# JerryX1110/Robust-Video-Object-Segmentation

Hardware: AMD Instinct MI355X
Metric: frames/sec, AOC-Net matching + calibration hot path (480p, 3 objects) (higher is better)
Workload: dtype f32; 1 GPU; cfg2: 121x213 stride-4 maps (480p), O=4 (3 objects + background), K=16 proxies, C=100, 60-frame clips, MEM_EVERY=5 (pool R=1..12), 20 Lloyd iterations, local windows 2..12, 10 IA gates + 4 conditioning blocks; sequences_per_gpu=2, proxy_mode=reference

## Files before the change

include/aoc_hip.h:

```cpp
#ifndef AOC_HIP_H
#define AOC_HIP_H

#include <stddef.h>
#include <stdint.h>

#ifdef __cplusplus
extern "C" {
#endif

typedef void *aoc_stream_t;

enum aoc_status {
    AOC_OK = 0,
    AOC_ERR_INVALID_ARG = -1,
    AOC_ERR_WORKSPACE = -2,
    AOC_ERR_LAUNCH = -3,
    AOC_ERR_UNSUPPORTED = -4
};

#define AOC_MAX_OBJECTS 30
#define AOC_MAX_CHANNELS 256
#define AOC_MAX_CLUSTERS 64
#define AOC_PAD_DISTANCE 5.0e4f
#define AOC_ROW_KEPT_BIT 0x80000000u
// ... 149 lines not shown
                              int transform, void *workspace, size_t workspace_bytes, aoc_stream_t stream);
int aoc_dense_match_min_split_cached(const float *query, const void *query_rec, const float *query_sqnorm, int query_rec_tiled,
                              int64_t m, int C, const float *pool, const void *pool_rec,
                              const int32_t *overflow_flag, int64_t n,
                              const uint32_t *right_bits, const uint32_t *wrong_bits,
                              const int32_t *fg_rows, const int32_t *obj_rows,
                              const int32_t *counts, const int32_t *obj_offsets,
                              const float *obj_bias, int n_obj,
                              float *out, int64_t out_pixel_stride, int64_t out_obj_stride,
                              int transform, void *workspace, size_t workspace_bytes, int reuse_plan, aoc_stream_t stream);

int aoc_dense_prune_stats(uint64_t *out4, int reset);
int aoc_dense_prune_stats_ex(uint64_t *out8, int reset);

int aoc_set_stream_cus(int n_cus);

int aoc_dense_match_set_probe(void *start_event, void *stop_event);

int aoc_local_window_match(const float *query, const float *prev, const uint32_t *right_bits,
                           int H, int W, int C, const int32_t *radii_host, int n_radii,
                           const float *obj_bias, int n_obj, float *out, int transform,
                           aoc_stream_t stream);

int aoc_local_window_match_ex(const float *query, const float *prev, const uint32_t *right_bits,
                              int H, int W, int C, const int32_t *radii_host, int n_radii,
                              const float *obj_bias, int n_obj, float *out, int transform,
                              int atrous_rate, int float16, aoc_stream_t stream);

int aoc_resize_bilinear_hwc(const float *in, int h, int w, int C, float *out, int H, int W,
                            aoc_stream_t stream);
// ... 332 lines not shown
```

robust-video-object-segmentation_amd/_lib.py:

```python
import ctypes
import os
import subprocess

_HERE = os.path.dirname(os.path.abspath(__file__))
CSRC = os.path.join(_HERE, "csrc")
RELEASE_SO = os.path.join(CSRC, "libaoc_hip.so")
if os.environ.get("AOC_LIB_VARIANT", "release") != "release":
    raise ImportError(f"AOC_LIB_VARIANT={os.environ['AOC_LIB_VARIANT']!r}: the development build and its switches are gone (commit fb2052a is the last "
                      "one that has them); unset the variable, or load a variant library of your own with AOC_LIB_FILE")
SO_PATH = RELEASE_SO
if os.environ.get("AOC_LIB_FILE"):
    SO_PATH = os.path.join(CSRC, os.environ["AOC_LIB_FILE"])

_vp, _i, _i64, _sz, _f = ctypes.c_void_p, ctypes.c_int, ctypes.c_int64, ctypes.c_size_t, ctypes.c_float

SIGNATURES = {
    "aoc_version": (ctypes.c_char_p, []),
    "aoc_label_prep_workspace_bytes": (_sz, [_i64, _i]),
    "aoc_label_prep": (_i, [_vp, _i64, _i, _vp, _vp, _vp, _vp, _vp, _vp, _vp, _sz, _vp]),
    "aoc_label_bits": (_i, [_vp, _i64, _i, _vp, _vp, _vp]),
    "aoc_kmeans_plan": (_i, [_vp, _i, _i, _vp, _vp]),
    "aoc_kmeans_init_rows_draw": (_i, [_vp, _vp, _vp, _i, _vp, _i, _i, _i, _vp, _vp]),
    "aoc_kmeans_workspace_bytes": (_sz, [_i64, _i, _i, _i]),
    "aoc_kmeans_segmented": (_i, [_vp, _i, _vp, _vp, _vp, _vp, _i, _i, _i, _i64, _vp, _vp, _vp, _vp, _sz, _vp]),
# ... 14 lines not shown
    "aoc_kmeans_replicate_levels": (_i, [_vp, _vp, _i, _i, _vp, _i, _i64, _vp, _vp, _vp, _vp]),
    "aoc_build_proxies_workspace_bytes": (_sz, [_i64, _i, _i]),
    "aoc_build_proxies": (_i, [_vp, _i64, _i, _vp, _vp, _vp, _vp, _vp, _i, _i, _i64, _vp, _vp, _vp, _sz, _vp]),
    "aoc_proxy_corr_min": (_i, [_vp, _i64, _i, _vp, _vp, _i, _i, _vp, _vp, _vp, _vp, _vp, _i64, _i, _vp]),
    "aoc_proxy_corr_min_batched_workspace_bytes": (_sz, []),
    "aoc_proxy_corr_min_batched": (_i, [_vp, _i, _i64, _i, _i, _i, _vp, _vp, _vp, _i, _i, _vp, _sz, _vp]),
    "aoc_proxy_corr_min_records": (_i, [_vp, _i, _i64, _i, _i, _i, _vp, _vp, _vp, _i, _vp, _sz, _vp]),
    "aoc_proxy_corr_min_records_cached_workspace_bytes": (_sz, []),
    "aoc_proxy_corr_min_records_cached": (_i, [_vp, _i, _i64, _i, _i, _i, _vp, _vp, _vp, _i, _vp, _sz, _vp, _vp]),
    "aoc_dense_match_workspace_bytes": (_sz, [_i64, _i64, _i]),
    "aoc_dense_match_min": (_i, [_vp, _i64, _i, _vp, _vp, _vp, _i64, _vp, _vp, _i, _vp, _i64, _i64, _i, _vp, _sz, _vp]),
    "aoc_dense_match_min_f16": (_i, [_vp, _i64, _i, _vp, _vp, _vp, _i64, _vp, _vp, _i, _vp, _i64, _i64, _i, _vp, _sz, _vp]),
    "aoc_proxy_corr_min_f16": (_i, [_vp, _i64, _i, _vp, _vp, _i, _i, _vp, _vp, _vp, _vp, _vp, _i64, _i, _vp]),
    "aoc_dense_match_set_probe": (_i, [_vp, _vp]),
    "aoc_set_stream_cus": (_i, [_i]),
    "aoc_split_record_bytes": (_sz, [_i]),
    "aoc_split_rows": (_i, [_vp, _i64, _i, _vp, _vp, _vp, _vp]),
    "aoc_split_rows_tiled_bytes": (_sz, [_i64, _i]),
    "aoc_split_rows_tiled": (_i, [_vp, _i64, _i, _vp, _vp, _vp, _vp]),
    "aoc_dense_match_split_workspace_bytes": (_sz, [_i64, _i64, _i]),
    "aoc_dense_prune_stats": (_i, [_vp, _i]),
    "aoc_dense_prune_stats_ex": (_i, [_vp, _i]),
    "aoc_dense_match_min_split": (_i, [_vp, _vp, _vp, _i, _i64, _i, _vp, _vp, _vp, _i64, _vp, _vp, _vp, _vp, _vp, _vp, _vp, _i, _vp, _i64, _i64, _i,
                                       _vp, _sz, _vp]),
    "aoc_dense_match_min_split_cached": (_i, [_vp, _vp, _vp, _i, _i64, _i, _vp, _vp, _vp, _i64, _vp, _vp, _vp, _vp, _vp, _vp, _vp, _i, _vp, _i64, _i64, _i,
                                              _vp, _sz, _i, _vp]),
    "aoc_frame_channels": (_i, [_i, _i, _i]),
    "aoc_frame_workspace_bytes": (_sz, [_i, _i, _i, _i, _i, _i, _i]),
    "aoc_frame_enqueue": (_i, [_vp, _vp, _vp, _sz, _vp]),
    "aoc_cluster_chain_workspace_bytes": (_sz, [_vp]),
# ... 136 lines not shown
```

robust-video-object-segmentation_amd/csrc/dense_split.hip:

```cpp
#include <atomic>
#include <type_traits>

#include "aoc_common.h"

namespace {

typedef _Float16 f16x8 __attribute__((ext_vector_type(8)));
typedef float f32x16 __attribute__((ext_vector_type(16)));

constexpr int SP_KS = 7;
constexpr int SP_K = SP_KS * 16;
constexpr int SP_HALF = SP_KS * 2;
constexpr int SP_REC = 2 * SP_HALF;
constexpr int SP_NORM_SLOT = 100;
constexpr float SP_SCALE = 1024.0f;
constexpr float SP_QCONST = 32768.0f;
constexpr float SP_UNSCALE = -1.0f / 524288.0f;
constexpr int SP_TILE = 32;
constexpr int SP_NB_HI = 8;
constexpr int SP_NQ = 2;
constexpr int SP_NW = 8;
constexpr int64_t SP_ROWS_PER_BLOCK = SP_NW * SP_NQ * 32;

static_assert(SP_NORM_SLOT + 4 <= SP_K && SP_NORM_SLOT / 16 == SP_KS - 1 && (SP_NORM_SLOT % 16) + 4 <= 8, "norm slots live in the low half of the last k-step");
// ... 180 lines not shown
constexpr int SP_CHUNK_BYTES = SP_NB_HI * SP_TILE_BYTES;
constexpr int SP_IDS_SLOTS = 3, SP_IDS_SLOT_BYTES = 1024;
constexpr int SP_IDS_OFF = SP_NBUF * SP_CHUNK_BYTES;
constexpr int SP_OBJ_OFF = SP_IDS_OFF + SP_IDS_SLOTS * SP_IDS_SLOT_BYTES;
constexpr int SP_BND_OFF = SP_OBJ_OFF + 4 * 256;
constexpr int SP_LDS_BYTES = SP_BND_OFF + SP_NW * SP_NQ * 256;
static_assert(SP_NQ == 2 && SP_NW == 8 && SP_NB_HI == 8 && SP_LDS_BYTES == 122880,
              "the step structure of dense_prune_kernel is written for 8 hi-plane tiles x 2 query tiles x 8 waves; 120 KiB per workgroup");
constexpr int SP_TILE_SLACK = 2;

template <int PLACE>
__global__ __launch_bounds__(SP_NW * 64, 1) void dense_prune_kernel(const uint4 *__restrict__ qrec, const float *__restrict__ q2, int64_t m,
                                                                     const uint4 *__restrict__ prec, const int32_t *__restrict__ tile_rows,
                                                                     const int32_t *__restrict__ tile_obj, const int32_t *__restrict__ n_tiles_ptr,
                                                                     const int32_t *__restrict__ gate, const uint32_t *__restrict__ pmax_bits,
                                                                     int n_obj, uint32_t *__restrict__ gbest, int q_tiled) {
    if (*gate) return;
    extern __shared__ __attribute__((aligned(16))) uint4 lds4[];
    constexpr int SWZ_MASK = 1;
    constexpr int SP_DMA_PER_WAVE = SP_CHUNK_BYTES / 1024 / SP_NW;
    constexpr int W_ID0 = SP_NW / 2, W_OBJ = 1;
    const uint32_t lds_base = (uint32_t)reinterpret_cast<uintptr_t>(lds4);
    const char *lds_bytes = reinterpret_cast<const char *>(lds4);

    int bx, by;
    {
        const int nb = gridDim.x * gridDim.y, lin = blockIdx.y * gridDim.x + blockIdx.x;
        const int xcd = lin & 7, slot = lin >> 3, q = nb >> 3, r = nb & 7;
        const int v = (xcd < r ? xcd * (q + 1) : r * (q + 1) + (xcd - r) * q) + slot;
        by = v / gridDim.x;
        bx = v - by * gridDim.x;
    }
    const int n_tiles = *n_tiles_ptr;
    const int ns = gridDim.y;
    if (by >= n_tiles) return;
    const int n_mine = (n_tiles - by + ns - 1) / ns;
    const int n_chunks = (n_mine + SP_NB_HI - 1) / SP_NB_HI;

    const int lane = aoc_lane(), wave = __builtin_amdgcn_readfirstlane(threadIdx.x >> 6);
    const int col = lane & 31, h = lane >> 5;
    const int64_t wave_row0 = (int64_t)bx * (SP_NW * SP_NQ * 32) + (int64_t)wave * (SP_NQ * 32);

    const float pmax = sqrtf(__uint_as_float(*pmax_bits)) * 1.001f;
    const float plmax = __uint_as_float(*(pmax_bits - 2));
    f16x8 bh[SP_NQ][SP_KS], bl[SP_NQ][SP_KS];
    float eps[SP_NQ];
    bool valid[SP_NQ];
#pragma unroll
    for (int iq = 0; iq < SP_NQ; ++iq) {
        const int64_t row = wave_row0 + iq * 32 + col;
        valid[iq] = row < m;
        const int64_t rr = valid[iq] ? row : 0;
        const uint4 *r = q_tiled ? qrec + (size_t)(rr >> 5) * (2 * SP_KS * 64) + h * 32 + (rr & 31) : qrec + (size_t)rr * SP_REC + h;
        const int ks_step = q_tiled ? 64 : 2, plane_step = q_tiled ? SP_KS * 64 : SP_HALF;
#pragma unroll
        for (int ks = 0; ks < SP_KS; ++ks) {
            uint4 u = r[ks * ks_step], v = r[plane_step + ks * ks_step];
            if (!valid[iq]) { u = make_uint4(0, 0, 0, 0); v = make_uint4(0, 0, 0, 0); }
            bh[iq][ks] = __builtin_bit_cast(f16x8, u);
            bl[iq][ks] = __builtin_bit_cast(f16x8, v);
        }
        const float ql_own = (float)bh[iq][SP_KS - 1][SP_NORM_SLOT % 16 + 3];
        if (h == 0) {
            bh[iq][SP_KS - 1][SP_NORM_SLOT % 16 + 3] = (_Float16)0.0f;
            bh[iq][SP_KS - 1][SP_NORM_SLOT % 16] = (_Float16)SP_QCONST;
            bh[iq][SP_KS - 1][SP_NORM_SLOT % 16 + 1] = (_Float16)SP_QCONST;
            bh[iq][SP_KS - 1][SP_NORM_SLOT % 16 + 2] = (_Float16)SP_QCONST;
        } else {
            bh[iq][SP_KS - 1][0] = (_Float16)0.0f;
            bh[iq][SP_KS - 1][1] = (_Float16)0.0f;
        }
        const float qn = valid[iq] ? sqrtf(q2[row]) : 0.0f;
        const float ql = valid[iq] ? __shfl(ql_own, col) : 0.0f;
        eps[iq] = 1026.0f * (qn * plmax + ql * pmax) + 8.0f * pmax * pmax + 0.0f + 8.0f;
    }

    uint32_t dma_plan[SP_DMA_PER_WAVE];
#pragma unroll
    for (int k = 0; k < SP_DMA_PER_WAVE; ++k) {
        const int j = (wave * SP_DMA_PER_WAVE + k) * 64 + lane;
        const int r = j / SP_ROW_CHUNKS, pos = j - r * SP_ROW_CHUNKS;
        dma_plan[k] = ((uint32_t)r << 16) | (uint32_t)((pos ^ ((r >> 3) & SWZ_MASK)) * 16);
    }
    const char *prec_bytes = reinterpret_cast<const char *>(prec);
    auto dma_meta = [&](int chunk) {
        const int i0 = chunk * SP_NB_HI;
        if (wave == W_ID0) {
            const int t = min(by + (i0 + (lane >> 3)) * ns, n_tiles);
            glds16(tile_rows + (size_t)t * SP_TILE + (lane & 7) * 4, lds_base + SP_IDS_OFF + (chunk % SP_IDS_SLOTS) * SP_IDS_SLOT_BYTES);
        }
        if (wave == W_OBJ) glds4(tile_obj + min(by + (i0 + (lane & (SP_NB_HI - 1))) * ns, n_tiles), lds_base + SP_OBJ_OFF + (chunk & 3) * 256);
    };
    auto dma_rows = [&](int chunk) {
        const int32_t *ids = reinterpret_cast<const int32_t *>(lds_bytes + SP_IDS_OFF + (chunk % SP_IDS_SLOTS) * SP_IDS_SLOT_BYTES);
        const uint32_t dst = lds_base + (uint32_t)(chunk % SP_NBUF) * SP_CHUNK_BYTES + (uint32_t)(wave * SP_DMA_PER_WAVE) * 1024u;
        int id[SP_DMA_PER_WAVE];
#pragma unroll
        for (int k = 0; k < SP_DMA_PER_WAVE; ++k) id[k] = ids[dma_plan[k] >> 16];
#pragma unroll
        for (int k = 0; k < SP_DMA_PER_WAVE; ++k)
            glds16(prec_bytes + (size_t)(uint32_t)max(id[k], 0) * (SP_REC * 16) + (dma_plan[k] & 0xffffu), dst + (uint32_t)k * 1024u);
    };

    float best[SP_NQ], shared[SP_NQ];
    uint32_t grow[SP_NQ];
#pragma unroll
    for (int iq = 0; iq < SP_NQ; ++iq) {
        grow[iq] = valid[iq] ? (uint32_t)(wave_row0 + iq * 32 + col) * (uint32_t)n_obj : 0u;
        best[iq] = INFINITY;
        shared[iq] = INFINITY;
    }
    int cur = -1;
    unsigned n_rescored = 0, n_any = 0, n_seen = 0;
    auto dma_bound = [&]() {
#pragma unroll
        for (int iq = 0; iq < SP_NQ; ++iq) {
            unsigned keep;
            asm volatile("s_mov_b32 %0, m0\n\ts_mov_b32 m0, %2\n\ts_nop 0\n\tglobal_load_lds_dword %1, off sc1\n\ts_mov_b32 m0, %0"
                         : "=&s"(keep) : "v"(gbest + grow[iq] + max(cur, 0)), "s"(lds_base + SP_BND_OFF + (uint32_t)(wave * SP_NQ + iq) * 256u) : "memory");
        }
    };
    auto switch_object = [&](int o) {
        cur = o;
        uint32_t u[SP_NQ];
#pragma unroll
        for (int iq = 0; iq < SP_NQ; ++iq) u[iq] = load_relaxed(gbest + grow[iq] + cur);
#pragma unroll
        for (int iq = 0; iq < SP_NQ; ++iq) {
            best[iq] = valid[iq] ? -INFINITY : INFINITY;
            shared[iq] = valid[iq] ? ord_dec(u[iq]) : INFINITY;
        }
    };

    dma_meta(0);
    dma_meta(1);
    __builtin_amdgcn_s_waitcnt(0x0f70);
    __builtin_amdgcn_s_barrier();
    dma_rows(0);
    __builtin_amdgcn_s_waitcnt(0x0f70);
    __builtin_amdgcn_s_barrier();

    const int xs = (col >> 3) & SWZ_MASK;
    const uint32_t row_off = (uint32_t)col * SP_ROW_BYTES;
    const uint32_t sw0 = row_off + (uint32_t)((h ^ xs) * 16), sw2 = sw0 + 32u;
    auto frag = [&](const char *tile_base, int e) -> f16x8 {
        const uint32_t off = ((e & 2) ? sw2 : sw0) + (uint32_t)((e & ~3) * 16);
        return __builtin_bit_cast(f16x8, *reinterpret_cast<const uint4 *>(tile_base + off));
    };
    auto ks_of = [&](int kk) { return (kk + SP_KS - 1) % SP_KS; };

    for (int s = 0; s < n_chunks; ++s) {
        const int4 objs = *reinterpret_cast<const int4 *>(lds_bytes + SP_OBJ_OFF + (s & 3) * 256);
        const int4 objs_b = *reinterpret_cast<const int4 *>(lds_bytes + (s & 3) * 256 + SP_OBJ_OFF + 16);
        const int bound_obj = cur;
        dma_bound();
        dma_meta(s + 2);
        dma_rows(s + 1);

        const char *chunk_base = lds_bytes + (s % SP_NBUF) * SP_CHUNK_BYTES;
        const int n_here = min(SP_NB_HI, n_mine - s * SP_NB_HI);
        f16x8 pre0 = frag(chunk_base, 2 * ks_of(0)), pre1 = frag(chunk_base, 2 * ks_of(1));
        const uint32_t objs_lo = (uint32_t)__builtin_amdgcn_readfirstlane((objs.x & 0xff) | ((objs.y & 0xff) << 8) | ((objs.z & 0xff) << 16) | ((objs.w & 0xff) << 24));
        const uint32_t objs_hi = (uint32_t)__builtin_amdgcn_readfirstlane((objs_b.x & 0xff) | ((objs_b.y & 0xff) << 8) | ((objs_b.z & 0xff) << 16) | ((objs_b.w & 0xff) << 24));
        const uint64_t objs_packed = ((uint64_t)objs_hi << 32) | objs_lo;
        const int32_t *ids_now = reinterpret_cast<const int32_t *>(lds_bytes + SP_IDS_OFF + (s % SP_IDS_SLOTS) * SP_IDS_SLOT_BYTES);
#pragma unroll 1
        for (int t = 0; t < n_here; ++t) {
            const char *tile_base = chunk_base + t * SP_TILE_BYTES;
            const int o = (int)((objs_packed >> (8 * t)) & 0xffu);
            if (o != cur) switch_object(o);
            f32x16 acc[SP_NQ];
#pragma unroll
            for (int iq = 0; iq < SP_NQ; ++iq)
#pragma unroll
                for (int r = 0; r < 16; ++r) acc[iq][r] = 0.0f;
            {
                f16x8 af[3];
                af[0] = pre0;
                af[1] = pre1;
#pragma unroll
                for (int kk = 0; kk < SP_KS; ++kk) {
                    if (kk + 2 < SP_KS) af[(kk + 2) % 3] = frag(tile_base, 2 * ks_of(kk + 2));
#pragma unroll
                    for (int iq = 0; iq < SP_NQ; ++iq)
                        acc[iq] = __builtin_amdgcn_mfma_f32_32x32x16_f16(af[kk % 3], bh[iq][ks_of(kk)], acc[iq], 0, 0, 0);
                }
                if (t + 1 < n_here) {
                    pre0 = frag(tile_base + SP_TILE_BYTES, 2 * ks_of(0));
                    pre1 = frag(tile_base + SP_TILE_BYTES, 2 * ks_of(1));
                }
            }
            bool want[SP_NQ];
#pragma unroll
            for (int iq = 0; iq < SP_NQ; ++iq) {
                const float cm = max16(acc[iq]);
                want[iq] = __builtin_amdgcn_ballot_w64(cm + eps[iq] >= __builtin_fmaxf(best[iq], shared[iq])) != 0ull;
            }
            n_seen += 1;
            if (want[0] || want[1]) {
                n_any += 1;
                f16x8 alg[SP_KS];
                auto load_lo = [&]() {
                    const int id = ids_now[t * SP_TILE + col];
                    const uint4 *lo = reinterpret_cast<const uint4 *>(prec_bytes + (size_t)(uint32_t)max(id, 0) * (SP_REC * 16) + SP_HALF * 16) + h;
#pragma unroll
                    for (int kk = 0; kk < SP_KS; ++kk) alg[kk] = __builtin_bit_cast(f16x8, lo[2 * ks_of(kk)]);
                    __builtin_amdgcn_s_waitcnt(0x0f70);
                };
                auto rescore = [&](auto iq_c) {
                    constexpr int iq = decltype(iq_c)::value;
                    n_rescored += 1;
                    f16x8 ah[3];
#pragma unroll
                    for (int kk = 0; kk < 2; ++kk) ah[kk] = frag(tile_base, 2 * ks_of(kk));
#pragma unroll
                    for (int kk = 0; kk < SP_KS; ++kk) {
                        if (kk + 2 < SP_KS) ah[(kk + 2) % 3] = frag(tile_base, 2 * ks_of(kk + 2));
                        acc[iq] = __builtin_amdgcn_mfma_f32_32x32x16_f16(ah[kk % 3], bl[iq][ks_of(kk)], acc[iq], 0, 0, 0);
                        acc[iq] = __builtin_amdgcn_mfma_f32_32x32x16_f16(alg[kk], bh[iq][ks_of(kk)], acc[iq], 0, 0, 0);
                    }
                    const float ex = max16(acc[iq]);
                    if (ex > best[iq]) {
                        best[iq] = ex;
                        if (ex > shared[iq]) atomicMax(gbest + grow[iq] + cur, ord_enc(ex));
                    }
                };
                load_lo();
                if (want[0]) rescore(std::integral_constant<int, 0>{});
                if (want[1]) rescore(std::integral_constant<int, 1>{});
            }
        }

        __builtin_amdgcn_s_waitcnt(0x0f70);
        uint32_t seen[SP_NQ];
#pragma unroll
        for (int iq = 0; iq < SP_NQ; ++iq)
            seen[iq] = *reinterpret_cast<const volatile uint32_t *>(lds_bytes + SP_BND_OFF + (wave * SP_NQ + iq) * 256 + lane * 4);
        __builtin_amdgcn_s_waitcnt(0xc07f);
        __builtin_amdgcn_s_barrier();
        if (bound_obj == cur && cur >= 0) {
#pragma unroll
            for (int iq = 0; iq < SP_NQ; ++iq)
                if (valid[iq]) shared[iq] = __builtin_fmaxf(shared[iq], ord_dec(seen[iq]));
        }
    }
    if (lane == 0) {
        atomicAdd(&g_prune_stats[0], (unsigned long long)n_seen * SP_NQ);
        atomicAdd(&g_prune_stats[1], (unsigned long long)n_rescored);
        atomicAdd(&g_prune_stats[2], (unsigned long long)n_any);
        atomicAdd(&g_prune_stats[3], (unsigned long long)n_seen);
        atomicAdd(&g_prune_stats[4], 0ull);
    }
}

constexpr int AOC_DENSE_SEED_FRAMES = 1;
__global__ __launch_bounds__(256) void dense_seed_kernel(const float *__restrict__ query, const float *__restrict__ q2, int64_t m, int C,
                                                          const float *__restrict__ pool, int64_t n, const uint32_t *__restrict__ right_bits, int n_obj,
                                                          const int32_t *__restrict__ gate, uint32_t *__restrict__ gbest) {
    if (*gate) return;
    const int sub = threadIdx.x & 7;
    const int64_t i = ((int64_t)blockIdx.x * blockDim.x + threadIdx.x) >> 3;
// ... 55 lines not shown
#pragma unroll
            for (int o2 = 0; o2 < 16; ++o2)
                if (o2 != o && o2 < n_obj) others = fminf(others, own[o2]);
            float v = fminf(own[o], others + AOC_PAD_DISTANCE);
            if (n_kept == 0) v = transform ? 1.0f : INFINITY;
            else if (transform) v = aoc_proto_transform(v, obj_bias ? obj_bias[o] : 0.0f);
            out[row * pstride + o * ostride] = v;
        }
    }
}

__global__ void split_gate_refresh_kernel(const int32_t *__restrict__ overflow, int32_t *__restrict__ gate) {
    if (*overflow) atomicOr(gate, 1);
}

inline int split_nsplit(int64_t m) {
    const int64_t row_blocks = (m + SP_ROWS_PER_BLOCK - 1) / SP_ROWS_PER_BLOCK;
    constexpr int max_rounds = 2;
    const int n_cu = aoc_stream_cus() > 0 ? aoc_stream_cus() : 256;
    int best = 1;
    double best_eff = 0.0;
    for (int k = 1; k <= max_rounds; ++k) {
        int64_t ns = ((int64_t)n_cu * k) / row_blocks;
        if (ns < 1) ns = 1;
        if (ns > 64) ns = 64;
        const int64_t blocks = row_blocks * ns;
        const int64_t rounds = (blocks + n_cu - 1) / n_cu;
        const double eff = (double)blocks / ((double)n_cu * rounds);
        if (eff >= best_eff - 0.005) { best_eff = eff > best_eff ? eff : best_eff; best = (int)ns; }
    }
    return best;
}

struct SplitWs {
    int32_t *gate, *n_tiles, *tile_rows, *tile_obj;
    uint32_t *pmax, *gbest;
    void *fp32_ws;
    size_t fp32_bytes, total;
    int64_t tile_capacity;
};
inline SplitWs split_carve(void *base, int64_t m, int64_t n, int n_obj) {
    SplitWs w;
    char *p = static_cast<char *>(base);
    size_t off = 0;
    auto take = [&](size_t bytes) { char *r = p ? p + off : nullptr; off += aoc_align_up(bytes, 256); return r; };
    w.tile_capacity = (n + SP_TILE - 1) / SP_TILE + n_obj + SP_TILE_SLACK;
// ... 71 lines not shown
    hipStream_t st = aoc_hip_stream(stream);
    const SplitWs w = split_carve(workspace, m, n, n_obj);
    if (reuse_plan) {
        hipLaunchKernelGGL(split_gate_refresh_kernel, dim3(1), dim3(1), 0, st, overflow_flag, w.gate);
    } else {
        if (hipMemsetAsync(w.gate, 0, 16, st) != hipSuccess) return AOC_ERR_LAUNCH;
        if (hipMemsetAsync(w.gbest, 0, (size_t)m * n_obj * sizeof(uint32_t), st) != hipSuccess) return AOC_ERR_LAUNCH;
        const int64_t plan_threads = w.tile_capacity * SP_TILE > n ? w.tile_capacity * SP_TILE : n;
        hipLaunchKernelGGL(split_plan_kernel, dim3((unsigned)((plan_threads + 255) / 256)), dim3(256), 0, st, obj_rows, counts, obj_offsets, n_obj, n,
                           right_bits, wrong_bits, overflow_flag, static_cast<const uint4 *>(pool_rec), w.tile_capacity, w.tile_rows, w.tile_obj,
                           w.n_tiles, w.gate, w.pmax);
    }
    if (n >= m)
        hipLaunchKernelGGL(dense_seed_kernel, dim3((unsigned)((m * 8 + 255) / 256)), dim3(256), 0, st, query, query_sqnorm, m, C, pool, n, right_bits, n_obj, w.gate,
                           w.gbest);
    const dim3 grid((unsigned)((m + SP_ROWS_PER_BLOCK - 1) / SP_ROWS_PER_BLOCK), split_nsplit(m));
    const AocDenseProbe probe = aoc_take_dense_probe();
    static const bool lds_ok = hipFuncSetAttribute(reinterpret_cast<const void *>(dense_prune_kernel<0>), hipFuncAttributeMaxDynamicSharedMemorySize,
                                                   SP_LDS_BYTES) == hipSuccess;
    if (!lds_ok) return AOC_ERR_LAUNCH;
    if (probe.start) (void)hipEventRecord(probe.start, st);
    hipLaunchKernelGGL(dense_prune_kernel<0>, grid, dim3(SP_NW * 64), SP_LDS_BYTES, st, static_cast<const uint4 *>(query_rec), query_sqnorm, m,
                       static_cast<const uint4 *>(pool_rec), w.tile_rows, w.tile_obj, w.n_tiles, w.gate, w.pmax, n_obj, w.gbest, query_rec_tiled ? 1 : 0);
    if (probe.stop) (void)hipEventRecord(probe.stop, st);
    hipLaunchKernelGGL(dense_split_finalize_kernel, dim3((unsigned)((m + 255) / 256)), dim3(256), 0, st, w.gbest, m, n_obj, counts, w.gate,
                       query_sqnorm, obj_bias, out, out_pixel_stride, out_obj_stride, transform);
    AOC_RETURN_IF_LAUNCH_FAILED();
    return aoc_dense_match_min_gated(query, m, C, pool, fg_rows, counts + n_obj, n, wrong_bits, obj_bias, n_obj, out, out_pixel_stride,
                                     out_obj_stride, transform, w.fp32_ws, w.fp32_bytes, w.gate, stream);
}

static std::atomic<int> g_stream_cus{0};
int aoc_set_stream_cus(int n_cus) {
    if (n_cus < 0) return AOC_ERR_INVALID_ARG;
    g_stream_cus.store(n_cus, std::memory_order_relaxed);
    return AOC_OK;
}

int aoc_dense_prune_stats(uint64_t *out4, int reset) {
    if (!out4) return AOC_ERR_INVALID_ARG;
    uint64_t v[8];
    const int rc = aoc_dense_prune_stats_ex(v, reset);
    for (int i = 0; i < 4 && rc == AOC_OK; ++i) out4[i] = v[i];
    return rc;
}

int aoc_dense_prune_stats_ex(uint64_t *out8, int reset) {
    if (!out8) return AOC_ERR_INVALID_ARG;
    unsigned long long v[8] = {0, 0, 0, 0, 0, 0, 0, 0};
    if (hipMemcpyFromSymbol(v, HIP_SYMBOL(g_prune_stats), sizeof(v)) != hipSuccess) return AOC_ERR_LAUNCH;
// ... 18 lines not shown
```

robust-video-object-segmentation_amd/ops.py:

```python
import ctypes
import os

import numpy as np
import torch

from . import _lib

PAD_DISTANCE = 5e4
MAX_OBJECTS = 30


def _need_gpu(*tensors):
    for t in tensors:
        if t is not None and not t.is_cuda:
            raise _lib.AocHipError("aoc_amd operators run only on an MI355X device tensor (no CPU fallback); "
                                   f"got a tensor on {t.device}")


_TRAINABLE = {"global_matching_for_eval": "matching_train.global_matching", "global_matching_for_eval_proxy": "matching_train.global_matching_proxy",
              "local_matching": "local_train.local_matching", "local_matching_proxy": "local_train.local_matching_proxy",
              "global_matching_for_eval_cluster": "cluster_train.global_matching_cluster2",
              "foreground2background": "frontend_train.foreground2background",
              "calculate_attention_head_for_eval_p_m": "frontend_train.calculate_attention_head_p_m",
              "IA_gate": "gates_train.IA_gate", "GCT": "gates_train.GCT", "conditioning_layer": "gates_train.conditioning_layer",
# ... 571 lines not shown
    _span("dense_match_min_split: out", out, _dense_span(m, n_obj, out_pixel_stride, out_obj_stride))
    right_bits, wrong_bits, fg_rows, obj_rows, counts, obj_offsets = _prep_lists(prep)
    q_rec, q_sq, p_rec = query_split.records, query_split.sqnorm, pool_split.records
    _lib.check(L.aoc_dense_match_min_split(_p(query_flat), _p(q_rec), _p(q_sq), int(query_split.tiled), m, C, _p(pool),
                                           _p(p_rec),
                                           _p(flag), n, _p(right_bits), _p(wrong_bits), _p(fg_rows), _p(obj_rows),
                                           _p(counts), _p(obj_offsets), _p(obj_bias), n_obj, _p(out), int(out_pixel_stride),
                                           int(out_obj_stride), int(bool(transform)), _p(ws), ws.numel(), _stream()),
               "aoc_dense_match_min_split")
    return out


DENSE_PRECISION = os.environ.get("AOC_DENSE_PRECISION", "split")


def set_stream_cus(n_cus):
    _lib.check(_lib.lib().aoc_set_stream_cus(int(n_cus)), "aoc_set_stream_cus")


def dense_match(query_flat, pool, prep, obj_bias, out, out_pixel_stride, out_obj_stride, transform=True, precision=None,
                query_split=None, pool_split=None):
    precision = precision or DENSE_PRECISION
    if precision not in ("split", "fp32", "f16"):
        raise ValueError(f"unknown dense precision {precision!r}")
    C = query_flat.shape[1]
    _span("dense_match: out", out, _dense_span(query_flat.shape[0], prep.n_obj, out_pixel_stride, out_obj_stride))
    if precision == "f16":
        return dense_match_min(query_flat, pool, prep, obj_bias, out, out_pixel_stride, out_obj_stride, transform, float16=True)
    if precision == "fp32" or split_record_bytes(C) == 0 or prep.n_obj > 16:
        return dense_match_min(query_flat, pool, prep, obj_bias, out, out_pixel_stride, out_obj_stride, transform)
    if pool_split is None:
        pool_split = split_rows(pool[:prep.n])
# ... 933 lines not shown
```

Baseline: 443.8 frames/s.

## Make dense prune kernel persistent with grid sized to a share of CUs

Result: faster. 451.3 frames/s, median of 6 (+1.7%).

```diff
diff --git a/include/aoc_hip.h b/include/aoc_hip.h
--- a/include/aoc_hip.h
+++ b/include/aoc_hip.h
@@ -187,6 +187,11 @@
 int aoc_dense_prune_stats_ex(uint64_t *out8, int reset);
 
 int aoc_set_stream_cus(int n_cus);
+
+#define AOC_DENSE_SHARE_DEFAULT 224
+int aoc_set_dense_share(int share_256);
+int aoc_dense_share(void);
+int aoc_dense_split_sizing(int64_t m, int budget, int share_256, int32_t *splits, int32_t *items, int32_t *workgroups);
 
 int aoc_dense_match_set_probe(void *start_event, void *stop_event);
 
diff --git a/robust-video-object-segmentation_amd/_lib.py b/robust-video-object-segmentation_amd/_lib.py
--- a/robust-video-object-segmentation_amd/_lib.py
+++ b/robust-video-object-segmentation_amd/_lib.py
@@ -52,6 +52,9 @@
     "aoc_proxy_corr_min_f16": (_i, [_vp, _i64, _i, _vp, _vp, _i, _i, _vp, _vp, _vp, _vp, _vp, _i64, _i, _vp]),
     "aoc_dense_match_set_probe": (_i, [_vp, _vp]),
     "aoc_set_stream_cus": (_i, [_i]),
+    "aoc_set_dense_share": (_i, [_i]),
+    "aoc_dense_share": (_i, []),
+    "aoc_dense_split_sizing": (_i, [_i64, _i, _i, _vp, _vp, _vp]),
     "aoc_split_record_bytes": (_sz, [_i]),
     "aoc_split_rows": (_i, [_vp, _i64, _i, _vp, _vp, _vp, _vp]),
     "aoc_split_rows_tiled_bytes": (_sz, [_i64, _i]),
diff --git a/robust-video-object-segmentation_amd/csrc/dense_split.hip b/robust-video-object-segmentation_amd/csrc/dense_split.hip
--- a/robust-video-object-segmentation_amd/csrc/dense_split.hip
+++ b/robust-video-object-segmentation_amd/csrc/dense_split.hip
@@ -218,7 +218,7 @@
                                                                      const uint4 *__restrict__ prec, const int32_t *__restrict__ tile_rows,
                                                                      const int32_t *__restrict__ tile_obj, const int32_t *__restrict__ n_tiles_ptr,
                                                                      const int32_t *__restrict__ gate, const uint32_t *__restrict__ pmax_bits,
-                                                                     int n_obj, uint32_t *__restrict__ gbest, int q_tiled) {
+                                                                     int n_obj, uint32_t *__restrict__ gbest, int q_tiled, int n_split) {
     if (*gate) return;
     extern __shared__ __attribute__((aligned(16))) uint4 lds4[];
     constexpr int SWZ_MASK = 1;
@@ -227,228 +227,233 @@
     const uint32_t lds_base = (uint32_t)reinterpret_cast<uintptr_t>(lds4);
     const char *lds_bytes = reinterpret_cast<const char *>(lds4);
 
-    int bx, by;
-    {
-        const int nb = gridDim.x * gridDim.y, lin = blockIdx.y * gridDim.x + blockIdx.x;
-        const int xcd = lin & 7, slot = lin >> 3, q = nb >> 3, r = nb & 7;
-        const int v = (xcd < r ? xcd * (q + 1) : r * (q + 1) + (xcd - r) * q) + slot;
-        by = v / gridDim.x;
-        bx = v - by * gridDim.x;
-    }
     const int n_tiles = *n_tiles_ptr;
-    const int ns = gridDim.y;
-    if (by >= n_tiles) return;
-    const int n_mine = (n_tiles - by + ns - 1) / ns;
-    const int n_chunks = (n_mine + SP_NB_HI - 1) / SP_NB_HI;
-
-    const int lane = aoc_lane(), wave = __builtin_amdgcn_readfirstlane(threadIdx.x >> 6);
-    const int col = lane & 31, h = lane >> 5;
-    const int64_t wave_row0 = (int64_t)bx * (SP_NW * SP_NQ * 32) + (int64_t)wave * (SP_NQ * 32);
-
-    const float pmax = sqrtf(__uint_as_float(*pmax_bits)) * 1.001f;
-    const float plmax = __uint_as_float(*(pmax_bits - 2));
-    f16x8 bh[SP_NQ][SP_KS], bl[SP_NQ][SP_KS];
-    float eps[SP_NQ];
-    bool valid[SP_NQ];
-#pragma unroll
-    for (int iq = 0; iq < SP_NQ; ++iq) {
-        const int64_t row = wave_row0 + iq * 32 + col;
-        valid[iq] = row < m;
-        const int64_t rr = valid[iq] ? row : 0;
-        const uint4 *r = q_tiled ? qrec + (size_t)(rr >> 5) * (2 * SP_KS * 64) + h * 32 + (rr & 31) : qrec + (size_t)rr * SP_REC + h;
-        const int ks_step = q_tiled ? 64 : 2, plane_step = q_tiled ? SP_KS * 64 : SP_HALF;
-#pragma unroll
-        for (int ks = 0; ks < SP_KS; ++ks) {
-            uint4 u = r[ks * ks_step], v = r[plane_step + ks * ks_step];
-            if (!valid[iq]) { u = make_uint4(0, 0, 0, 0); v = make_uint4(0, 0, 0, 0); }
-            bh[iq][ks] = __builtin_bit_cast(f16x8, u);
-            bl[iq][ks] = __builtin_bit_cast(f16x8, v);
-        }
-        const float ql_own = (float)bh[iq][SP_KS - 1][SP_NORM_SLOT % 16 + 3];
-        if (h == 0) {
-            bh[iq][SP_KS - 1][SP_NORM_SLOT % 16 + 3] = (_Float16)0.0f;
-            bh[iq][SP_KS - 1][SP_NORM_SLOT % 16] = (_Float16)SP_QCONST;
-            bh[iq][SP_KS - 1][SP_NORM_SLOT % 16 + 1] = (_Float16)SP_QCONST;
-            bh[iq][SP_KS - 1][SP_NORM_SLOT % 16 + 2] = (_Float16)SP_QCONST;
-        } else {
-            bh[iq][SP_KS - 1][0] = (_Float16)0.0f;
-            bh[iq][SP_KS - 1][1] = (_Float16)0.0f;
-        }
-        const float qn = valid[iq] ? sqrtf(q2[row]) : 0.0f;
-        const float ql = valid[iq] ? __shfl(ql_own, col) : 0.0f;
-        eps[iq] = 1026.0f * (qn * plmax + ql * pmax) + 8.0f * pmax * pmax + 0.0f + 8.0f;
-    }
-
-    uint32_t dma_plan[SP_DMA_PER_WAVE];
-#pragma unroll
-    for (int k = 0; k < SP_DMA_PER_WAVE; ++k) {
-        const int j = (wave * SP_DMA_PER_WAVE + k) * 64 + lane;
-        const int r = j / SP_ROW_CHUNKS, pos = j - r * SP_ROW_CHUNKS;
-        dma_plan[k] = ((uint32_t)r << 16) | (uint32_t)((pos ^ ((r >> 3) & SWZ_MASK)) * 16);
-    }
-    const char *prec_bytes = reinterpret_cast<const char *>(prec);
-    auto dma_meta = [&](int chunk) {
-        const int i0 = chunk * SP_NB_HI;
-        if (wave == W_ID0) {
-            const int t = min(by + (i0 + (lane >> 3)) * ns, n_tiles);
-            glds16(tile_rows + (size_t)t * SP_TILE + (lane & 7) * 4, lds_base + SP_IDS_OFF + (chunk % SP_IDS_SLOTS) * SP_IDS_SLOT_BYTES);
-        }
-        if (wave == W_OBJ) glds4(tile_obj + min(by + (i0 + (lane & (SP_NB_HI - 1))) * ns, n_tiles), lds_base + SP_OBJ_OFF + (chunk & 3) * 256);
-    };
-    auto dma_rows = [&](int chunk) {
-        const int32_t *ids = reinterpret_cast<const int32_t *>(lds_bytes + SP_IDS_OFF + (chunk % SP_IDS_SLOTS) * SP_IDS_SLOT_BYTES);
-        const uint32_t dst = lds_base + (uint32_t)(chunk % SP_NBUF) * SP_CHUNK_BYTES + (uint32_t)(wave * SP_DMA_PER_WAVE) * 1024u;
-        int id[SP_DMA_PER_WAVE];
-#pragma unroll
-        for (int k = 0; k < SP_DMA_PER_WAVE; ++k) id[k] = ids[dma_plan[k] >> 16];
-#pragma unroll
-        for (int k = 0; k < SP_DMA_PER_WAVE; ++k)
-            glds16(prec_bytes + (size_t)(uint32_t)max(id[k], 0) * (SP_REC * 16) + (dma_plan[k] & 0xffffu), dst + (uint32_t)k * 1024u);
-    };
-
-    float best[SP_NQ], shared[SP_NQ];
-    uint32_t grow[SP_NQ];
-#pragma unroll
-    for (int iq = 0; iq < SP_NQ; ++iq) {
-        grow[iq] = valid[iq] ? (uint32_t)(wave_row0 + iq * 32 + col) * (uint32_t)n_obj : 0u;
-        best[iq] = INFINITY;
-        shared[iq] = INFINITY;
-    }
-    int cur = -1;
+    const int ns = n_split;
+    const int nbx = (int)((m + SP_ROWS_PER_BLOCK - 1) / SP_ROWS_PER_BLOCK), nb = nbx * ns;
+    const int wave = __builtin_amdgcn_readfirstlane(threadIdx.x >> 6);
     unsigned n_rescored = 0, n_any = 0, n_seen = 0;
-    auto dma_bound = [&]() {
+#pragma unroll 1
+    for (int lin = blockIdx.x; lin < nb; lin += gridDim.x) {
+        int lane = aoc_lane();
+        asm volatile("" : "+v"(lane));
+        const int col = lane & 31, h = lane >> 5;
+        const float pmax = sqrtf(__uint_as_float(*pmax_bits)) * 1.001f;
+        const float plmax = __uint_as_float(*(pmax_bits - 2));
+        int bx, by;
+        {
+            const int xcd = lin & 7, slot = lin >> 3, q = nb >> 3, r = nb & 7;
+            const int v = (xcd < r ? xcd * (q + 1) : r * (q + 1) + (xcd - r) * q) + slot;
+            by = v / nbx;
+            bx = v - by * nbx;
+        }
+        if (by >= n_tiles) continue;
+        const int n_mine = (n_tiles - by + ns - 1) / ns;
+        const int n_chunks = (n_mine + SP_NB_HI - 1) / SP_NB_HI;
+
+        const int64_t wave_row0 = (int64_t)bx * (SP_NW * SP_NQ * 32) + (int64_t)wave * (SP_NQ * 32);
+
+        f16x8 bh[SP_NQ][SP_KS], bl[SP_NQ][SP_KS];
+        float eps[SP_NQ];
+        bool valid[SP_NQ];
 #pragma unroll
         for (int iq = 0; iq < SP_NQ; ++iq) {
-            unsigned keep;
-            asm volatile("s_mov_b32 %0, m0\n\ts_mov_b32 m0, %2\n\ts_nop 0\n\tglobal_load_lds_dword %1, off sc1\n\ts_mov_b32 m0, %0"
-                         : "=&s"(keep) : "v"(gbest + grow[iq] + max(cur, 0)), "s"(lds_base + SP_BND_OFF + (uint32_t)(wave * SP_NQ + iq) * 256u) : "memory");
-        }
-    };
-    auto switch_object = [&](int o) {
-        cur = o;
-        uint32_t u[SP_NQ];
-#pragma unroll
-        for (int iq = 0; iq < SP_NQ; ++iq) u[iq] = load_relaxed(gbest + grow[iq] + cur);
+            const int64_t row = wave_row0 + iq * 32 + col;
+            valid[iq] = row < m;
+            const int64_t rr = valid[iq] ? row : 0;
+            const uint4 *r = q_tiled ? qrec + (size_t)(rr >> 5) * (2 * SP_KS * 64) + h * 32 + (rr & 31) : qrec + (size_t)rr * SP_REC + h;
+            const int ks_step = q_tiled ? 64 : 2, plane_step = q_tiled ? SP_KS * 64 : SP_HALF;
+#pragma unroll
+            for (int ks = 0; ks < SP_KS; ++ks) {
+                uint4 u = r[ks * ks_step], v = r[plane_step + ks * ks_step];
+                if (!valid[iq]) { u = make_uint4(0, 0, 0, 0); v = make_uint4(0, 0, 0, 0); }
+                bh[iq][ks] = __builtin_bit_cast(f16x8, u);
+                bl[iq][ks] = __builtin_bit_cast(f16x8, v);
+            }
+            const float ql_own = (float)bh[iq][SP_KS - 1][SP_NORM_SLOT % 16 + 3];
+            if (h == 0) {
+                bh[iq][SP_KS - 1][SP_NORM_SLOT % 16 + 3] = (_Float16)0.0f;
+                bh[iq][SP_KS - 1][SP_NORM_SLOT % 16] = (_Float16)SP_QCONST;
+                bh[iq][SP_KS - 1][SP_NORM_SLOT % 16 + 1] = (_Float16)SP_QCONST;
+                bh[iq][SP_KS - 1][SP_NORM_SLOT % 16 + 2] = (_Float16)SP_QCONST;
+            } else {
+                bh[iq][SP_KS - 1][0] = (_Float16)0.0f;
+                bh[iq][SP_KS - 1][1] = (_Float16)0.0f;
+            }
+            const float qn = valid[iq] ? sqrtf(q2[row]) : 0.0f;
+            const float ql = valid[iq] ? __shfl(ql_own, col) : 0.0f;
+            eps[iq] = 1026.0f * (qn * plmax + ql * pmax) + 8.0f * pmax * pmax + 0.0f + 8.0f;
+        }
+
+        uint32_t dma_plan[SP_DMA_PER_WAVE];
+#pragma unroll
+        for (int k = 0; k < SP_DMA_PER_WAVE; ++k) {
+            const int j = (wave * SP_DMA_PER_WAVE + k) * 64 + lane;
+            const int r = j / SP_ROW_CHUNKS, pos = j - r * SP_ROW_CHUNKS;
+            dma_plan[k] = ((uint32_t)r << 16) | (uint32_t)((pos ^ ((r >> 3) & SWZ_MASK)) * 16);
+        }
+        const char *prec_bytes = reinterpret_cast<const char *>(prec);
+        auto dma_meta = [&](int chunk) {
+            const int i0 = chunk * SP_NB_HI;
+            if (wave == W_ID0) {
+                const int t = min(by + (i0 + (lane >> 3)) * ns, n_tiles);
+                glds16(tile_rows + (size_t)t * SP_TILE + (lane & 7) * 4, lds_base + SP_IDS_OFF + (chunk % SP_IDS_SLOTS) * SP_IDS_SLOT_BYTES);
+            }
+            if (wave == W_OBJ) glds4(tile_obj + min(by + (i0 + (lane & (SP_NB_HI - 1))) * ns, n_tiles), lds_base + SP_OBJ_OFF + (chunk & 3) * 256);
+        };
+        auto dma_rows = [&](int chunk) {
+            const int32_t *ids = reinterpret_cast<const int32_t *>(lds_bytes + SP_IDS_OFF + (chunk % SP_IDS_SLOTS) * SP_IDS_SLOT_BYTES);
+            const uint32_t dst = lds_base + (uint32_t)(chunk % SP_NBUF) * SP_CHUNK_BYTES + (uint32_t)(wave * SP_DMA_PER_WAVE) * 1024u;
+            int id[SP_DMA_PER_WAVE];
+#pragma unroll
+            for (int k = 0; k < SP_DMA_PER_WAVE; ++k) id[k] = ids[dma_plan[k] >> 16];
+#pragma unroll
+            for (int k = 0; k < SP_DMA_PER_WAVE; ++k)
+                glds16(prec_bytes + (size_t)(uint32_t)max(id[k], 0) * (SP_REC * 16) + (dma_plan[k] & 0xffffu), dst + (uint32_t)k * 1024u);
+        };
+
+        float best[SP_NQ], shared[SP_NQ];
+        uint32_t grow[SP_NQ];
 #pragma unroll
         for (int iq = 0; iq < SP_NQ; ++iq) {
-            best[iq] = valid[iq] ? -INFINITY : INFINITY;
-            shared[iq] = valid[iq] ? ord_dec(u[iq]) : INFINITY;
-        }
-    };
-
-    dma_meta(0);
-    dma_meta(1);
-    __builtin_amdgcn_s_waitcnt(0x0f70);
-    __builtin_amdgcn_s_barrier();
-    dma_rows(0);
-    __builtin_amdgcn_s_waitcnt(0x0f70);
-    __builtin_amdgcn_s_barrier();
-
-    const int xs = (col >> 3) & SWZ_MASK;
-    const uint32_t row_off = (uint32_t)col * SP_ROW_BYTES;
-    const uint32_t sw0 = row_off + (uint32_t)((h ^ xs) * 16), sw2 = sw0 + 32u;
-    auto frag = [&](const char *tile_base, int e) -> f16x8 {
-        const uint32_t off = ((e & 2) ? sw2 : sw0) + (uint32_t)((e & ~3) * 16);
-        return __builtin_bit_cast(f16x8, *reinterpret_cast<const uint4 *>(tile_base + off));
-    };
-    auto ks_of = [&](int kk) { return (kk + SP_KS - 1) % SP_KS; };
-
-    for (int s = 0; s < n_chunks; ++s) {
-        const int4 objs = *reinterpret_cast<const int4 *>(lds_bytes + SP_OBJ_OFF + (s & 3) * 256);
-        const int4 objs_b = *reinterpret_cast<const int4 *>(lds_bytes + (s & 3) * 256 + SP_OBJ_OFF + 16);
-        const int bound_obj = cur;
-        dma_bound();
-        dma_meta(s + 2);
-        dma_rows(s + 1);
-
-        const char *chunk_base = lds_bytes + (s % SP_NBUF) * SP_CHUNK_BYTES;
-        const int n_here = min(SP_NB_HI, n_mine - s * SP_NB_HI);
-        f16x8 pre0 = frag(chunk_base, 2 * ks_of(0)), pre1 = frag(chunk_base, 2 * ks_of(1));
-        const uint32_t objs_lo = (uint32_t)__builtin_amdgcn_readfirstlane((objs.x & 0xff) | ((objs.y & 0xff) << 8) | ((objs.z & 0xff) << 16) | ((objs.w & 0xff) << 24));
-        const uint32_t objs_hi = (uint32_t)__builtin_amdgcn_readfirstlane((objs_b.x & 0xff) | ((objs_b.y & 0xff) << 8) | ((objs_b.z & 0xff) << 16) | ((objs_b.w & 0xff) << 24));
-        const uint64_t objs_packed = ((uint64_t)objs_hi << 32) | objs_lo;
-        const int32_t *ids_now = reinterpret_cast<const int32_t *>(lds_bytes + SP_IDS_OFF + (s % SP_IDS_SLOTS) * SP_IDS_SLOT_BYTES);
+            grow[iq] = valid[iq] ? (uint32_t)(wave_row0 + iq * 32 + col) * (uint32_t)n_obj : 0u;
+            best[iq] = INFINITY;
+            shared[iq] = INFINITY;
+        }
+        int cur = -1;
+        auto dma_bound = [&]() {
+#pragma unroll
+            for (int iq = 0; iq < SP_NQ; ++iq) {
+                unsigned keep;
+                asm volatile("s_mov_b32 %0, m0\n\ts_mov_b32 m0, %2\n\ts_nop 0\n\tglobal_load_lds_dword %1, off sc1\n\ts_mov_b32 m0, %0"
+                             : "=&s"(keep) : "v"(gbest + grow[iq] + max(cur, 0)), "s"(lds_base + SP_BND_OFF + (uint32_t)(wave * SP_NQ + iq) * 256u) : "memory");
+            }
+        };
+        auto switch_object = [&](int o) {
+            cur = o;
+            uint32_t u[SP_NQ];
+#pragma unroll
+            for (int iq = 0; iq < SP_NQ; ++iq) u[iq] = load_relaxed(gbest + grow[iq] + cur);
+#pragma unroll
+            for (int iq = 0; iq < SP_NQ; ++iq) {
+                best[iq] = valid[iq] ? -INFINITY : INFINITY;
+                shared[iq] = valid[iq] ? ord_dec(u[iq]) : INFINITY;
+            }
+        };
+
+        dma_meta(0);
+        dma_meta(1);
+        __builtin_amdgcn_s_waitcnt(0x0f70);
+        __builtin_amdgcn_s_barrier();
+        dma_rows(0);
+        __builtin_amdgcn_s_waitcnt(0x0f70);
+        __builtin_amdgcn_s_barrier();
+
+        const int xs = (col >> 3) & SWZ_MASK;
+        const uint32_t row_off = (uint32_t)col * SP_ROW_BYTES;
+        const uint32_t sw0 = row_off + (uint32_t)((h ^ xs) * 16), sw2 = sw0 + 32u;
+        auto frag = [&](const char *tile_base, int e) -> f16x8 {
+            const uint32_t off = ((e & 2) ? sw2 : sw0) + (uint32_t)((e & ~3) * 16);
+            return __builtin_bit_cast(f16x8, *reinterpret_cast<const uint4 *>(tile_base + off));
+        };
+        auto ks_of = [&](int kk) { return (kk + SP_KS - 1) % SP_KS; };
+
+        for (int s = 0; s < n_chunks; ++s) {
+            const int4 objs = *reinterpret_cast<const int4 *>(lds_bytes + SP_OBJ_OFF + (s & 3) * 256);
+            const int4 objs_b = *reinterpret_cast<const int4 *>(lds_bytes + (s & 3) * 256 + SP_OBJ_OFF + 16);
+            const int bound_obj = cur;
+            dma_bound();
+            dma_meta(s + 2);
+            dma_rows(s + 1);
+
+            const char *chunk_base = lds_bytes + (s % SP_NBUF) * SP_CHUNK_BYTES;
+            const int n_here = min(SP_NB_HI, n_mine - s * SP_NB_HI);
+            f16x8 pre0 = frag(chunk_base, 2 * ks_of(0)), pre1 = frag(chunk_base, 2 * ks_of(1));
+            const uint32_t objs_lo = (uint32_t)__builtin_amdgcn_readfirstlane((objs.x & 0xff) | ((objs.y & 0xff) << 8) | ((objs.z & 0xff) << 16) | ((objs.w & 0xff) << 24));
+            const uint32_t objs_hi = (uint32_t)__builtin_amdgcn_readfirstlane((objs_b.x & 0xff) | ((objs_b.y & 0xff) << 8) | ((objs_b.z & 0xff) << 16) | ((objs_b.w & 0xff) << 24));
+            const uint64_t objs_packed = ((uint64_t)objs_hi << 32) | objs_lo;
+            const int32_t *ids_now = reinterpret_cast<const int32_t *>(lds_bytes + SP_IDS_OFF + (s % SP_IDS_SLOTS) * SP_IDS_SLOT_BYTES);
 #pragma unroll 1
-        for (int t = 0; t < n_here; ++t) {
-            const char *tile_base = chunk_base + t * SP_TILE_BYTES;
-            const int o = (int)((objs_packed >> (8 * t)) & 0xffu);
-            if (o != cur) switch_object(o);
-            f32x16 acc[SP_NQ];
+            for (int t = 0; t < n_here; ++t) {
+                const char *tile_base = chunk_base + t * SP_TILE_BYTES;
+                const int o = (int)((objs_packed >> (8 * t)) & 0xffu);
+                if (o != cur) switch_object(o);
+                f32x16 acc[SP_NQ];
+#pragma unroll
+                for (int iq = 0; iq < SP_NQ; ++iq)
+#pragma unroll
+                    for (int r = 0; r < 16; ++r) acc[iq][r] = 0.0f;
+                {
+                    f16x8 af[3];
+                    af[0] = pre0;
+                    af[1] = pre1;
+#pragma unroll
+                    for (int kk = 0; kk < SP_KS; ++kk) {
+                        if (kk + 2 < SP_KS) af[(kk + 2) % 3] = frag(tile_base, 2 * ks_of(kk + 2));
+#pragma unroll
+                        for (int iq = 0; iq < SP_NQ; ++iq)
+                            acc[iq] = __builtin_amdgcn_mfma_f32_32x32x16_f16(af[kk % 3], bh[iq][ks_of(kk)], acc[iq], 0, 0, 0);
+                    }
+                    if (t + 1 < n_here) {
+                        pre0 = frag(tile_base + SP_TILE_BYTES, 2 * ks_of(0));
+                        pre1 = frag(tile_base + SP_TILE_BYTES, 2 * ks_of(1));
+                    }
+                }
+                bool want[SP_NQ];
+#pragma unroll
+                for (int iq = 0; iq < SP_NQ; ++iq) {
+                    const float cm = max16(acc[iq]);
+                    want[iq] = __builtin_amdgcn_ballot_w64(cm + eps[iq] >= __builtin_fmaxf(best[iq], shared[iq])) != 0ull;
+                }
+                n_seen += 1;
+                if (want[0] || want[1]) {
+                    n_any += 1;
+                    f16x8 alg[SP_KS];
+                    auto load_lo = [&]() {
+                        const int id = ids_now[t * SP_TILE + col];
+                        const uint4 *lo = reinterpret_cast<const uint4 *>(prec_bytes + (size_t)(uint32_t)max(id, 0) * (SP_REC * 16) + SP_HALF * 16) + h;
+#pragma unroll
+                        for (int kk = 0; kk < SP_KS; ++kk) alg[kk] = __builtin_bit_cast(f16x8, lo[2 * ks_of(kk)]);
+                        __builtin_amdgcn_s_waitcnt(0x0f70);
+                    };
+                    auto rescore = [&](auto iq_c) {
+                        constexpr int iq = decltype(iq_c)::value;
+                        n_rescored += 1;
+                        f16x8 ah[3];
+#pragma unroll
+                        for (int kk = 0; kk < 2; ++kk) ah[kk] = frag(tile_base, 2 * ks_of(kk));
+#pragma unroll
+                        for (int kk = 0; kk < SP_KS; ++kk) {
+                            if (kk + 2 < SP_KS) ah[(kk + 2) % 3] = frag(tile_base, 2 * ks_of(kk + 2));
+                            acc[iq] = __builtin_amdgcn_mfma_f32_32x32x16_f16(ah[kk % 3], bl[iq][ks_of(kk)], acc[iq], 0, 0, 0);
+                            acc[iq] = __builtin_amdgcn_mfma_f32_32x32x16_f16(alg[kk], bh[iq][ks_of(kk)], acc[iq], 0, 0, 0);
+                        }
+                        const float ex = max16(acc[iq]);
+                        if (ex > best[iq]) {
+                            best[iq] = ex;
+                            if (ex > shared[iq]) atomicMax(gbest + grow[iq] + cur, ord_enc(ex));
+                        }
+                    };
+                    load_lo();
+                    if (want[0]) rescore(std::integral_constant<int, 0>{});
+                    if (want[1]) rescore(std::integral_constant<int, 1>{});
+                }
+            }
+
+            __builtin_amdgcn_s_waitcnt(0x0f70);
+            uint32_t seen[SP_NQ];
 #pragma unroll
             for (int iq = 0; iq < SP_NQ; ++iq)
-#pragma unroll
-                for (int r = 0; r < 16; ++r) acc[iq][r] = 0.0f;
-            {
-                f16x8 af[3];
-                af[0] = pre0;
-                af[1] = pre1;
-#pragma unroll
-                for (int kk = 0; kk < SP_KS; ++kk) {
-                    if (kk + 2 < SP_KS) af[(kk + 2) % 3] = frag(tile_base, 2 * ks_of(kk + 2));
-#pragma unroll
-                    for (int iq = 0; iq < SP_NQ; ++iq)
-                        acc[iq] = __builtin_amdgcn_mfma_f32_32x32x16_f16(af[kk % 3], bh[iq][ks_of(kk)], acc[iq], 0, 0, 0);
-                }
-                if (t + 1 < n_here) {
-                    pre0 = frag(tile_base + SP_TILE_BYTES, 2 * ks_of(0));
-                    pre1 = frag(tile_base + SP_TILE_BYTES, 2 * ks_of(1));
-                }
-            }
-            bool want[SP_NQ];
-#pragma unroll
-            for (int iq = 0; iq < SP_NQ; ++iq) {
-                const float cm = max16(acc[iq]);
-                want[iq] = __builtin_amdgcn_ballot_w64(cm + eps[iq] >= __builtin_fmaxf(best[iq], shared[iq])) != 0ull;
-            }
-            n_seen += 1;
-            if (want[0] || want[1]) {
-                n_any += 1;
-                f16x8 alg[SP_KS];
-                auto load_lo = [&]() {
-                    const int id = ids_now[t * SP_TILE + col];
-                    const uint4 *lo = reinterpret_cast<const uint4 *>(prec_bytes + (size_t)(uint32_t)max(id, 0) * (SP_REC * 16) + SP_HALF * 16) + h;
-#pragma unroll
-                    for (int kk = 0; kk < SP_KS; ++kk) alg[kk] = __builtin_bit_cast(f16x8, lo[2 * ks_of(kk)]);
-                    __builtin_amdgcn_s_waitcnt(0x0f70);
-                };
-                auto rescore = [&](auto iq_c) {
-                    constexpr int iq = decltype(iq_c)::value;
-                    n_rescored += 1;
-                    f16x8 ah[3];
-#pragma unroll
-                    for (int kk = 0; kk < 2; ++kk) ah[kk] = frag(tile_base, 2 * ks_of(kk));
-#pragma unroll
-                    for (int kk = 0; kk < SP_KS; ++kk) {
-                        if (kk + 2 < SP_KS) ah[(kk + 2) % 3] = frag(tile_base, 2 * ks_of(kk + 2));
-                        acc[iq] = __builtin_amdgcn_mfma_f32_32x32x16_f16(ah[kk % 3], bl[iq][ks_of(kk)], acc[iq], 0, 0, 0);
-                        acc[iq] = __builtin_amdgcn_mfma_f32_32x32x16_f16(alg[kk], bh[iq][ks_of(kk)], acc[iq], 0, 0, 0);
-                    }
-                    const float ex = max16(acc[iq]);
-                    if (ex > best[iq]) {
-                        best[iq] = ex;
-                        if (ex > shared[iq]) atomicMax(gbest + grow[iq] + cur, ord_enc(ex));
-                    }
-                };
-                load_lo();
-                if (want[0]) rescore(std::integral_constant<int, 0>{});
-                if (want[1]) rescore(std::integral_constant<int, 1>{});
-            }
-        }
-
-        __builtin_amdgcn_s_waitcnt(0x0f70);
-        uint32_t seen[SP_NQ];
-#pragma unroll
-        for (int iq = 0; iq < SP_NQ; ++iq)
-            seen[iq] = *reinterpret_cast<const volatile uint32_t *>(lds_bytes + SP_BND_OFF + (wave * SP_NQ + iq) * 256 + lane * 4);
-        __builtin_amdgcn_s_waitcnt(0xc07f);
-        __builtin_amdgcn_s_barrier();
-        if (bound_obj == cur && cur >= 0) {
-#pragma unroll
-            for (int iq = 0; iq < SP_NQ; ++iq)
-                if (valid[iq]) shared[iq] = __builtin_fmaxf(shared[iq], ord_dec(seen[iq]));
-        }
-    }
-    if (lane == 0) {
+                seen[iq] = *reinterpret_cast<const volatile uint32_t *>(lds_bytes + SP_BND_OFF + (wave * SP_NQ + iq) * 256 + lane * 4);
+            __builtin_amdgcn_s_waitcnt(0xc07f);
+            __builtin_amdgcn_s_barrier();
+            if (bound_obj == cur && cur >= 0) {
+#pragma unroll
+                for (int iq = 0; iq < SP_NQ; ++iq)
+                    if (valid[iq]) shared[iq] = __builtin_fmaxf(shared[iq], ord_dec(seen[iq]));
+            }
+        }
+    }
+    if (aoc_lane() == 0) {
         atomicAdd(&g_prune_stats[0], (unsigned long long)n_seen * SP_NQ);
         atomicAdd(&g_prune_stats[1], (unsigned long long)n_rescored);
         atomicAdd(&g_prune_stats[2], (unsigned long long)n_any);
@@ -534,22 +539,33 @@
     if (*overflow) atomicOr(gate, 1);
 }
 
-inline int split_nsplit(int64_t m) {
+std::atomic<int> g_dense_share{AOC_DENSE_SHARE_DEFAULT};
+
+struct SplitSizing {
+    int splits, items, workgroups;
+};
+inline SplitSizing split_sizing(int64_t m, int budget, int share) {
     const int64_t row_blocks = (m + SP_ROWS_PER_BLOCK - 1) / SP_ROWS_PER_BLOCK;
-    constexpr int max_rounds = 2;
-    const int n_cu = aoc_stream_cus() > 0 ? aoc_stream_cus() : 256;
+    const int n_cu = budget > 0 ? budget : 256;
+    int64_t g = ((int64_t)n_cu * share) >> 8;
+    if (g >= 8) g &= ~(int64_t)7;
+    if (g < 1) g = 1;
+    const int max_rounds = share >= 256 ? 2 : 3;
     int best = 1;
     double best_eff = 0.0;
     for (int k = 1; k <= max_rounds; ++k) {
-        int64_t ns = ((int64_t)n_cu * k) / row_blocks;
+        int64_t ns = (g * k) / row_blocks;
         if (ns < 1) ns = 1;
         if (ns > 64) ns = 64;
         const int64_t blocks = row_blocks * ns;
-        const int64_t rounds = (blocks + n_cu - 1) / n_cu;
-        const double eff = (double)blocks / ((double)n_cu * rounds);
+        const int64_t rounds = (blocks + g - 1) / g;
+        const double eff = (double)blocks / ((double)g * rounds);
         if (eff >= best_eff - 0.005) { best_eff = eff > best_eff ? eff : best_eff; best = (int)ns; }
     }
-    return best;
+    const int64_t items = row_blocks * best;
+    if (g > items) g = items;
+    if (g >= 8) g &= ~(int64_t)7;
+    return SplitSizing{best, (int)items, (int)g};
 }
 
 struct SplitWs {
@@ -651,14 +667,16 @@
     if (n >= m)
         hipLaunchKernelGGL(dense_seed_kernel, dim3((unsigned)((m * 8 + 255) / 256)), dim3(256), 0, st, query, query_sqnorm, m, C, pool, n, right_bits, n_obj, w.gate,
                            w.gbest);
-    const dim3 grid((unsigned)((m + SP_ROWS_PER_BLOCK - 1) / SP_ROWS_PER_BLOCK), split_nsplit(m));
+    const SplitSizing sz = split_sizing(m, aoc_stream_cus(), g_dense_share.load(std::memory_order_relaxed));
+    const dim3 grid((unsigned)sz.workgroups);
     const AocDenseProbe probe = aoc_take_dense_probe();
     static const bool lds_ok = hipFuncSetAttribute(reinterpret_cast<const void *>(dense_prune_kernel<0>), hipFuncAttributeMaxDynamicSharedMemorySize,
                                                    SP_LDS_BYTES) == hipSuccess;
     if (!lds_ok) return AOC_ERR_LAUNCH;
     if (probe.start) (void)hipEventRecord(probe.start, st);
     hipLaunchKernelGGL(dense_prune_kernel<0>, grid, dim3(SP_NW * 64), SP_LDS_BYTES, st, static_cast<const uint4 *>(query_rec), query_sqnorm, m,
-                       static_cast<const uint4 *>(pool_rec), w.tile_rows, w.tile_obj, w.n_tiles, w.gate, w.pmax, n_obj, w.gbest, query_rec_tiled ? 1 : 0);
+                       static_cast<const uint4 *>(pool_rec), w.tile_rows, w.tile_obj, w.n_tiles, w.gate, w.pmax, n_obj, w.gbest, query_rec_tiled ? 1 : 0,
+                       sz.splits);
     if (probe.stop) (void)hipEventRecord(probe.stop, st);
     hipLaunchKernelGGL(dense_split_finalize_kernel, dim3((unsigned)((m + 255) / 256)), dim3(256), 0, st, w.gbest, m, n_obj, counts, w.gate,
                        query_sqnorm, obj_bias, out, out_pixel_stride, out_obj_stride, transform);
@@ -671,6 +689,22 @@
 int aoc_set_stream_cus(int n_cus) {
     if (n_cus < 0) return AOC_ERR_INVALID_ARG;
     g_stream_cus.store(n_cus, std::memory_order_relaxed);
+    return AOC_OK;
+}
+
+int aoc_set_dense_share(int share_256) {
+    if (share_256 < 1 || share_256 > 256) return AOC_ERR_INVALID_ARG;
+    g_dense_share.store(share_256, std::memory_order_relaxed);
+    return AOC_OK;
+}
+int aoc_dense_share(void) { return g_dense_share.load(std::memory_order_relaxed); }
+
+int aoc_dense_split_sizing(int64_t m, int budget, int share_256, int32_t *splits, int32_t *items, int32_t *workgroups) {
+    if (m < 1 || m >= (1ll << 31) || budget < 0 || share_256 < 1 || share_256 > 256 || !splits || !items || !workgroups) return AOC_ERR_INVALID_ARG;
+    const SplitSizing sz = split_sizing(m, budget, share_256);
+    *splits = sz.splits;
+    *items = sz.items;
+    *workgroups = sz.workgroups;
     return AOC_OK;
 }
 
diff --git a/robust-video-object-segmentation_amd/ops.py b/robust-video-object-segmentation_amd/ops.py
--- a/robust-video-object-segmentation_amd/ops.py
+++ b/robust-video-object-segmentation_amd/ops.py
@@ -609,8 +609,13 @@
 DENSE_PRECISION = os.environ.get("AOC_DENSE_PRECISION", "split")
 
 
-def set_stream_cus(n_cus):
-    _lib.check(_lib.lib().aoc_set_stream_cus(int(n_cus)), "aoc_set_stream_cus")
+def set_stream_cus(n_cus=None, dense_share=None):
+    L = _lib.lib()
+    if n_cus is not None:
+        _lib.check(L.aoc_set_stream_cus(int(n_cus)), "aoc_set_stream_cus")
+    if dense_share is not None:
+        _lib.check(L.aoc_set_dense_share(int(dense_share)), "aoc_set_dense_share")
+    return int(L.aoc_dense_share())
 
 
 def dense_match(query_flat, pool, prep, obj_bias, out, out_pixel_stride, out_obj_stride, transform=True, precision=None,
```
